# imuncle/TSCM_Calib

Hardware: AMD Instinct MI355X
Metric: LM iterations/sec at 4 cams x 10k views (joint intrinsics+extrinsics, fp64) (higher is better)
Workload: dtype f64

## Files before the change

### tscm_calib_amd/csrc/tscm_kernels.h

```cpp
#pragma once

#include "tscm_math.h"
#include "tscm_fastmath.h"
#include "tscm_nd_plan.h"
#include "tscm_layout.h"
#include "tscm_exec_plan.h"
#include "tscm_columns.h"

namespace tscm {

static_assert(kColFree == kFA && kColGrad == kFR, "tscm_columns.h plans the columns of tscm_math.h's camera tile");
constexpr int kWcolTc = 3;
constexpr int kFac = 56;
constexpr int kFacM = 0;
constexpr int kFacC = 15;
constexpr int kFacL = 21;
constexpr int kFacI = 36;
constexpr int kFacZ = 42;
constexpr int kFacD = 48;
constexpr int kTcols = 15;
constexpr int kTcWb = 0, kTcWc = 4, kTcF = 8, kTcOne = 9, kTcXi = 10, kTcLam = 12, kTcAl = 13, kTcR = 14;
__host__ __device__ constexpr int tc_tc(int j) { return 3 + 4 * j; }
constexpr int kVConst = 27;
constexpr int kCConst = 48;
// ... 58 lines not shown
    default: __builtin_amdgcn_s_setprio(3); break;
    }
}

__device__ __forceinline__ const double *rec_w(const double *rec, int slot) { return rec + (size_t)kRecW * slot; }
__device__ __forceinline__ const double *rec_e(const double *rec, int V, int slot) { return rec + (size_t)kRecW * V + (size_t)kRecE * slot; }
__device__ __forceinline__ const double *rec_g(const double *rec, int V, int slot) { return rec + (size_t)(kRecW + kRecE) * V + (size_t)kRecG * slot; }

struct Options {
    int max_num_iterations;
    double function_tolerance, gradient_tolerance, parameter_tolerance;
    double initial_radius, max_radius, min_radius;
    double min_relative_decrease, min_lm_diagonal, max_lm_diagonal;
    int max_invalid;
    int jacobi_scaling;
};

struct IterLog {
    int iteration, step_is_valid, step_is_successful, pad;
    double cost, cost_change, gradient_max_norm, gradient_norm, step_norm, relative_decrease, radius;
};

enum TermReason { kNone = 0, kMaxIter, kGradTol, kMinRadius, kParamTol, kFuncTol, kInvalidSteps };

struct CtrlHead {
    int done, term_type, term_reason, iteration;
    int cur, lin_fail, num_successful, num_unsuccessful;
    int num_invalid, n_log, lm_iterations, fin_count;
    int fault, pad0;
    double radius, decrease_factor;
    double x_cost, x_norm, gmax, gnorm;
    double model_cam, stepsq_cam;
    double se_min, se_cur, se_ref, se_cand, se_acc_ref, se_acc_cand;
    double initial_cost;
    Options opt;
    long long t_begin, t_end;
};

struct Ctrl : CtrlHead {
    IterLog log[kMaxLog];
};

struct DevProblem {
    int C, B, n_points, V, N, n_pad;
    int n_chunks, n_pchunks, n_bids;
    int rp, half;
    int lds_wave;
    const double *board_xy;
    const int *view_cam, *view_board, *view_obs, *view_count;
    const double *obs_u, *obs_v;
    const int *chunk_vb, *chunk_ve, *chunk_cam, *cam_chunk_ptr;
    const int4 *chunk_desc;
    const int *bv_ptr;
    const int *view_slot, *slot_cam;
    const int *slot_view, *slot_board;
    const int *slow_boards;
    int n_slow;
    const int *pair_i, *pair_j;
    const int *pc_begin, *pc_end, *pc_tile;
    const int *bid_part_ptr;
    const int *pair_board;
    const int *bc_tile;
    const int4 *bc_desc;
    int n_bchunks, n_tiles;
    const unsigned char *col_ctl;
    const unsigned char *board_const;
    const unsigned char *col_active;
    const int *act_map;
    int n_act;
    int cam_pre[9];
    unsigned short cam_free[8];
    unsigned long long pair_mask;
    const int4 *solve_map;
    int cam_wg[9];
    int rank, world;
    const short *bid_lut;
    int bid_part_small[kSmallBids + 1];
    int g4_per;
};

struct DevState {
    double *cam_rt[2], *intr[2], *board_rt[2];
    double *board_pc, *cam_pc;
    double *vconst;
    double *cconst[2];
    double *rec[2];
    double *campart, *campart2;
    double *H[2], *H_stage;
    double *s_b, *s_c;
    double *fac;
    double *pairpart, *T;
    int *t_count;
    int *fac_fail;
    int *y_flag;
    double *yhat;
    double *Abig;
    double *bs_part, *st_part;
    int n_bs_blocks, n_st_blocks;
    Ctrl *ctrl;
    CtrlHead *ctrl_snap;
    int *stats_count, *stats_flag;
    struct CtlPub *ctl_pub;
};
struct CtlPub { int epoch, cur, done, pad; double radius; };

__global__ void k_pose_prep(DevProblem P, DevState S, int cand)
{
    if (S.ctrl->done) return;
    const int tgt = cand ? (S.ctrl->cur ^ 1) : S.ctrl->cur;
    const int i = blockIdx.x * blockDim.x + threadIdx.x;
    if (i < P.B) {
        double rt[6], out[kBoardConst];
        for (int k = 0; k < 6; ++k) rt[k] = S.board_rt[tgt][6 * i + k];
        board_constants(rt, out);
        for (int k = 0; k < kBoardConst; ++k) S.board_pc[(size_t)kBoardConst * i + k] = out[k];
    } else if (i < P.B + P.C) {
        const int m = i - P.B;
        double rt[6], out[kCamConst];
        for (int k = 0; k < 6; ++k) rt[k] = S.cam_rt[tgt][6 * m + k];
        camera_constants(rt, out);
        for (int k = 0; k < kCamConst; ++k) S.cam_pc[kCamConst * m + k] = out[k];
    }
}

__device__ __forceinline__ void load_view_const(const DevProblem &P, const DevState &S, int tgt, int cam, int board, ViewConst &vc)
{
    const double *bp = S.board_pc + (size_t)kBoardConst * board;
    for (int k = 0; k < 3; ++k) { vc.r1[k] = bp[k]; vc.r2[k] = bp[3 + k]; vc.tb[k] = S.board_rt[tgt][6 * board + 3 + k]; }
    for (int k = 0; k < 3; ++k) for (int q = 0; q < 6; ++q) vc.db[k][q] = bp[6 + 6 * k + q];
    const double *cp = S.cam_pc + kCamConst * cam;
    for (int k = 0; k < 9; ++k) vc.Rc[k] = cp[k];
    for (int k = 0; k < 27; ++k) vc.dRc[k] = cp[9 + k];
    for (int k = 0; k < 3; ++k) vc.tc[k] = S.cam_rt[tgt][6 * cam + 3 + k];
    const double *I = S.intr[tgt] + 9 * cam;
    vc.fx = I[0]; vc.fy = I[1]; vc.cx = I[2]; vc.cy = I[3]; vc.xi = I[4]; vc.lam = I[5]; vc.al = I[6];
}

__device__ __forceinline__ void view_point_constants(const double Rc[9], const double *tc, const double *bc , const double *tb, double *o)
{
    for (int r = 0; r < 3; ++r) {
        o[r] = Rc[3 * r] * bc[0] + Rc[3 * r + 1] * bc[1] + Rc[3 * r + 2] * bc[2];
        o[3 + r] = Rc[3 * r] * bc[3] + Rc[3 * r + 1] * bc[4] + Rc[3 * r + 2] * bc[5];
        o[6 + r] = (Rc[3 * r] * tb[0] + Rc[3 * r + 1] * tb[1] + Rc[3 * r + 2] * tb[2]) + tc[r];
    }
}

#if defined(__HIP_DEVICE_COMPILE__) && !defined(__gfx950__) && !defined(__gfx942__)
#error "the in-launch hand-offs (handoff_store / handoff_load) rely on gfx942 / gfx950 sc1 write-through semantics: re-derive them for this target"
#endif
constexpr long long kHandoffTimeoutTicks = 50 * 1000 * 1000;
__device__ __forceinline__ void handoff_store(double *p, double v) { __hip_atomic_store(p, v, __ATOMIC_RELAXED, __HIP_MEMORY_SCOPE_AGENT); }
__device__ __forceinline__ double handoff_load(const double *p) { return __hip_atomic_load(p, __ATOMIC_RELAXED, __HIP_MEMORY_SCOPE_AGENT); }

__device__ __forceinline__ void write_camera_record(const DevState &S, int tgt, int m, const double *cam_rt, const double *intr)
{
    double crt[3], Rc[9], a[9], wsm[3];
    for (int k = 0; k < 3; ++k) crt[k] = cam_rt[6 * m + k];
    const int small = camera_rotation_constants(crt, Rc, a, wsm);
    double *o = S.cconst[tgt] + kCStride * m;
    for (int k = 0; k < 9; ++k) o[k] = Rc[k];
    for (int k = 0; k < 3; ++k) o[9 + k] = cam_rt[6 * m + 3 + k];
    for (int k = 0; k < 9; ++k) o[12 + k] = a[k];
    for (int k = 0; k < 3; ++k) o[21 + k] = wsm[k];
    o[24] = small ? 1.0 : 0.0;
    for (int k = 25; k < 39; ++k) o[k] = 0.0;
    double I[7];
    for (int k = 0; k < 7; ++k) I[k] = intr[9 * m + k];
    for (int k = 0; k < 6; ++k) o[39 + k] = I[k];
    const double oma = 1.0 - I[6];
    o[45] = I[6] / oma;
    o[46] = 1.0 / (oma * oma);
    o[47] = 0.0;
    float *of = reinterpret_cast<float *>(o + kCConst);
    for (int k = 0; k < kCConst; ++k) of[k] = (float)o[k];
}
__device__ __forceinline__ void write_camera_record(const DevState &S, int tgt, int m) { write_camera_record(S, tgt, m, S.cam_rt[tgt], S.intr[tgt]); }

constexpr int kVStride = 48;
constexpr int kVFloatOff = 32;
constexpr int kVPrepThreads = 128;

__device__ __forceinline__ void view_prep_body(const DevProblem &P, const DevState &S, int tgt, int with_floats, const double *cam_rt, const double *intr, const double *board_rt)
{
    __shared__ double st[kVPrepThreads][kVFloatOff + 1];
    const int t = threadIdx.x;
    const int i = blockIdx.x * kVPrepThreads + t;
    if (i < P.V) {
        const int b = P.view_board[i], m = P.view_cam[i];
        double rt[6], bc[kBoardConst], Rc[9], dRc[27];
        for (int k = 0; k < 6; ++k) rt[k] = board_rt[6 * b + k];
        board_constants(rt, bc);
        double crt[3];
        for (int k = 0; k < 3; ++k) crt[k] = cam_rt[6 * m + k];
        rotation_and_derivatives(crt, Rc, dRc);
        double *o = st[t];
        view_point_constants(Rc, cam_rt + 6 * m + 3, bc, rt + 3, o);
        for (int k = 0; k < 6; ++k) {
            const double d0 = bc[6 + 3 * k], d1 = bc[6 + 3 * k + 1], d2 = bc[6 + 3 * k + 2];
            for (int r = 0; r < 3; ++r) o[9 + 3 * k + r] = Rc[3 * r] * d0 + Rc[3 * r + 1] * d1 + Rc[3 * r + 2] * d2;
        }
        for (int k = kVConst; k < kVFloatOff; ++k) o[k] = 0.0;
    } else if (i < P.V + P.C) {
        write_camera_record(S, tgt, i - P.V, cam_rt, intr);
    }
    __syncthreads();
    const int v0 = blockIdx.x * kVPrepThreads;
    const int nv = min(kVPrepThreads, P.V - v0);
    for (int e = t; e < nv * kVFloatOff; e += kVPrepThreads) {
        const int v = e / kVFloatOff, k = e % kVFloatOff;
        S.vconst[(size_t)kVStride * (v0 + v) + k] = st[v][k];
    }
    if (with_floats) {
        constexpr int kF = kVStride - kVFloatOff;
        for (int e = t; e < nv * kF; e += kVPrepThreads) {
            const int v = e / kF, k = e % kF, j = 2 * k;
            const float f0 = j < kVConst ? (float)st[v][j] : 0.f, f1 = j + 1 < kVConst ? (float)st[v][j + 1] : 0.f;
            S.vconst[(size_t)kVStride * (v0 + v) + kVFloatOff + k] = __hiloint2double(__float_as_int(f1), __float_as_int(f0));
        }
    }
}

__global__ __launch_bounds__(kVPrepThreads) void k_view_prep(DevProblem P, DevState S, int cand, int with_floats)
{
    if (S.ctrl->done) return;
    const int tgt = cand ? (S.ctrl->cur ^ 1) : S.ctrl->cur;
    view_prep_body(P, S, tgt, with_floats, S.cam_rt[tgt], S.intr[tgt], S.board_rt[tgt]);
}

__host__ __device__ __forceinline__ constexpr int f_tile(int f)
{
    return f < 3 ? kTcWc + f : f < 6 ? tc_tc(f - 3) : f < 8 ? kTcF : f < 10 ? kTcOne : f == 10 ? kTcXi : f == 11 ? kTcLam : f == 12 ? kTcAl : kTcR;
}
__device__ __forceinline__ int f_mask(int f) { return (f >= 6 && f < 10) ? (1 << ((f - 6) & 1)) : 3; }

typedef const double __attribute__((address_space(4))) *cptr4;

struct RecLane { unsigned off, stride, goff, gstride; };
__device__ __forceinline__ RecLane rec_lane(int lane, unsigned V)
{
    const int col = lane & 15, kq = lane >> 4;
    RecLane r;
    r.goff = col == kTcR ? 8u * ((unsigned)(kRecW + kRecE) * V + (unsigned)kq) : 0xffffe000u; r.gstride = col == kTcR ? 8u * kRecG : 0u;
    if (col < 3) { r.off = 8u * ((unsigned)kRecW * V + 6u * (unsigned)col + (unsigned)kq); r.stride = 8u * kRecE; }
    else if (col == 15) { r.off = 0xffffe000u; r.stride = 0u; }
    else {
        const int f = (col & 3) == 3 ? kWcolTc + (col >> 2) : col < 8 ? col - kTcWc : col == kTcF ? 6 : col == kTcOne ? 8 : col == kTcXi ? 10 : col - 1;
        r.off = 8u * (6u * (unsigned)f + (unsigned)kq); r.stride = 8u * kRecW;
    }
    return r;
}

template <typename PW, typename PR>
__host__ __device__ __forceinline__ double tb_tb(PW W, PR Rc, int l, int lp)
{
    double t = Rc[3 + lp] * W[6 * (kWcolTc + 1) + 3 + l];
    t = fma(Rc[lp], W[6 * kWcolTc + 3 + l], t);
    return fma(Rc[6 + lp], W[6 * (kWcolTc + 2) + 3 + l], t);
}

__device__ __forceinline__ void store_view_record(__amdgpu_buffer_rsrc_t r_rec, int lane, const d4 &accU, const d4 &accV, cptr4 cc, unsigned slot, RecLane rl)
{
    int le = lane;
    asm volatile("" : "+v"(le));
    const int col = le & 15;
    const bool k3 = le >= 48, split = col == kTcF || col == kTcOne;
    constexpr unsigned BAD = 0xffffe000u;
    const unsigned off = rl.off + __umul24(slot, rl.stride);
    const double t0 = accU[0] + accV[0], t1 = accU[1] + accV[1], t2 = accU[2] + accV[2];
    double tbT[3], tbU[3];
#pragma unroll
    for (int l = 0; l < 3; ++l) {
        tbT[l] = fma(cc[6 + l], t2, fma(cc[l], t0, cc[3 + l] * t1));
        tbU[l] = fma(cc[6 + l], accU[2], fma(cc[l], accU[0], cc[3 + l] * accU[1]));
    }
    const double selT = k3 ? tbT[0] : t0, selU = k3 ? tbU[0] : accU[0];
    buf_store_f64(r_rec, off, 0u, split ? selU : selT);
    buf_store_2f64(r_rec, (k3 ? off : BAD) + 8u, split ? tbU[1] : tbT[1], split ? tbU[2] : tbT[2]);
    buf_store_f64(r_rec, (split ? off : BAD) + 48u, 0u, selT - selU);
    buf_store_2f64(r_rec, (split && k3 ? off : BAD) + 56u, tbT[1] - tbU[1], tbT[2] - tbU[2]);
    const unsigned og = rl.goff + __umul24(slot, rl.gstride);
    buf_store_f64(r_rec, og, 0u, selT);
    buf_store_2f64(r_rec, (k3 ? og : BAD) + 8u, tbT[1], tbT[2]);
}


enum GCol { gcWb0 = 0, gcWb1, gcWb2, gcTc0, gcTc1, gcTc2, gcWc0, gcWc1, gcWc2, gcF, gcOne, gcXi, gcLam, gcAl, gcR };

template <typename FV, typename FC, typename FP>
__device__ __forceinline__ void corner_geometry(double x, double y, double ou, double ov, FV VC, FC CC, FP PUT)
{
    const double X = fma(x, VC(0), fma(y, VC(3), VC(6)));
    const double Y = fma(x, VC(1), fma(y, VC(4), VC(7)));
    const double Z = fma(x, VC(2), fma(y, VC(5), VC(8)));
    const double fx = CC(39), fy = CC(40), xi = CC(43), lam = CC(44), beta = CC(45);
    const double rho2 = X * X + Y * Y;
    double d1, id1, d2, id2, d3, id3;
    sqrt_and_inverse(rho2 + Z * Z, d1, id1);
    const double z1 = Z + xi * d1;
    sqrt_and_inverse(rho2 + z1 * z1, d2, id2);
    const double z2 = z1 + lam * d2;
    sqrt_and_inverse(rho2 + z2 * z2, d3, id3);
    const double k = z2 + beta * d3;
    const double ik = fast_rcp(k);
    const double mx = X * ik, my = Y * ik;
    const double c1 = 1.0 + xi * Z * id1;
    const double c2 = 1.0 + lam * z1 * id2;
    const double c3 = 1.0 + beta * z2 * id3;
    const double q = beta * id3 + c3 * (lam * id2 + c2 * xi * id1);
    const double kz = c1 * c2 * c3;
    const double fxk = fx * ik, fyk = fy * ik;
    const double n00 = -fxk * (1.0 - X * mx * q), n01 = fxk * mx * Y * q, n02 = fxk * mx * kz;
    const double n10 = fyk * my * X * q, n11 = -fyk * (1.0 - Y * my * q), n12 = fyk * my * kz;
    PUT(gcTc0, n00, n10);
    PUT(gcTc1, n01, n11);
    PUT(gcTc2, n02, n12);
#pragma unroll
    for (int kk = 0; kk < 3; ++kk) {
        const double h0 = x * VC(9 + 6 * kk) + y * VC(12 + 6 * kk);
        const double h1 = x * VC(10 + 6 * kk) + y * VC(13 + 6 * kk);
        const double h2 = x * VC(11 + 6 * kk) + y * VC(14 + 6 * kk);
        PUT(gcWb0 + kk, n00 * h0 + n01 * h1 + n02 * h2, n10 * h0 + n11 * h1 + n12 * h2);
    }
    {
        double Q0 = X - CC(9), Q1 = Y - CC(10), Q2 = Z - CC(11);
        if (CC(24) != 0.0) {
            const double w0 = CC(21), w1 = CC(22), w2 = CC(23);
            const double s0 = w1 * Q2 - w2 * Q1, s1 = w2 * Q0 - w0 * Q2, s2 = w0 * Q1 - w1 * Q0;
// ... 1080 lines not shown
        if (!factor_core(M, g, sb, radius, dmin, dmax, facl[tid], board_is_const)) *S.fac_fail = 1;
    }
    __syncthreads();
    PHASE_STAMP(ts2);
    for (int i = tid; i < nbd * kFac; i += 256) S.fac[(size_t)kFac * c0 + i] = (&facl[0][0])[i];
    d4 acc[NT];
#pragma unroll
    for (int t = 0; t < NT; ++t) acc[t] = d4{ 0.0, 0.0, 0.0, 0.0 };
    const bool grad_col = a == kFR;
#pragma unroll
    for (int g = 0; g < 4; ++g) {
        if (16 * wave + 4 * g >= nbd) break;
        const int bg = 16 * wave + 4 * g + kq;
        const bool valid = bg < nbd;
        const int bl = min(bg, nbd - 1);
        FacFwd F;
#pragma unroll
        for (int i = 0; i < 15; ++i) F.m[i] = facl[bl][kFacM + i];
#pragma unroll
        for (int i = 0; i < 6; ++i) { F.c[i] = facl[bl][kFacC + i]; F.z[i] = valid ? facl[bl][kFacZ + i] : 0.0; }
        double y[NV][6];
#pragma unroll
        for (int p = 0; p < NV; ++p) y_column(F, w[g][p], grad_col, y[p]);
#pragma unroll
        for (int r = 0; r < 6; ++r) {
            int t = 0;
#pragma unroll
            for (int p = 0; p < NV; ++p)
#pragma unroll
                for (int q = p; q < NV; ++q, ++t) acc[t] = __builtin_amdgcn_mfma_f64_16x16x4f64(y[p][r], y[q][r], acc[t], 0, 0, 0);
        }
    }
    PHASE_STAMP(ts3);
#pragma unroll
    for (int t = 0; t < NT; ++t)
#pragma unroll
        for (int r = 0; r < 4; ++r) tiles[wave][t][(kq + 4 * r) * 16 + a] = acc[t][r];
    __syncthreads();
#pragma unroll
    for (int t = 0; t < NT; ++t)
        S.pairpart[(size_t)256 * P.bc_tile[6 * chunk + t] + tid] = (tiles[0][t][tid] + tiles[1][t][tid]) + (tiles[2][t][tid] + tiles[3][t][tid]);
#ifdef TSCM_WAVE_TIMELINE
    if (threadIdx.x == 0 && ktl_scope.on && (int)blockIdx.x < kKtlGroups) {
        long long *o = g_phs + (size_t)kPhStamps * blockIdx.x;
        o[0] = tsk; o[1] = ts0; o[2] = ts1; o[3] = ts2; o[4] = ts3; o[5] = wall_clock64(); o[6] = nbd; o[7] = (bid >= first_round ? 1 : 0) | ((RIDE && t_waited ? t_waited - tsk : 0) << 1) | ((RIDE && t_reduced ? t_reduced - tsk : 0) << 32);
    }
#endif
#ifdef TSCM_PHASE_PROFILE
    if (threadIdx.x == 0 && (cblk == 0 || cblk == 200))
        printf("schur_gram wg %d: boards %d  head %lld  E sums %lld  factor %lld  gram %lld  tiles %lld [10 ns]\n", (int)blockIdx.x, nbd, ts0 - tsk, ts1 - ts0, ts2 - ts1, ts3 - ts2, wall_clock64() - ts3);
#endif
}

__global__ __launch_bounds__(256) void k_pair_gram(DevProblem P, DevState S)
{
    if (S.ctrl->done) return;
    __shared__ double red[4][256];
    const int pc = blockIdx.x;
    const int cur = S.ctrl->cur;
    const int wave = threadIdx.x >> 6, lane = threadIdx.x & 63;
    const int a = lane & 15, kq = lane >> 4;
    d4 acc = { 0.0, 0.0, 0.0, 0.0 };
    for (int p = P.pc_begin[pc] + wave; p < P.pc_end[pc]; p += 4) {
        const double *Wi = rec_w(S.rec[cur], P.pair_i[p]), *Wj = rec_w(S.rec[cur], P.pair_j[p]);
        FacFwd F;
        load_fac_fwd(S.fac, __builtin_amdgcn_readfirstlane(P.pair_board[p]), F);
        double wi[6], wj[6];
#pragma unroll
        for (int k = 0; k < 6; ++k) { wi[k] = a < 14 ? Wi[6 * a + k] : 0.0; wj[k] = a < 14 ? Wj[6 * a + k] : 0.0; }
        double i0, i1, j0, j1;
        y_column_operands(F, wi, a == kFR, kq, i0, i1);
        y_column_operands(F, wj, a == kFR, kq, j0, j1);
        acc = __builtin_amdgcn_mfma_f64_16x16x4f64(i0, j0, acc, 0, 0, 0);
        acc = __builtin_amdgcn_mfma_f64_16x16x4f64(i1, j1, acc, 0, 0, 0);
    }
#pragma unroll
    for (int r = 0; r < 4; ++r) red[wave][(kq + 4 * r) * 16 + a] = acc[r];
    __syncthreads();
    const int t = threadIdx.x;
    S.pairpart[(size_t)256 * P.pc_tile[pc] + t] = (red[0][t] + red[1][t]) + (red[2][t] + red[3][t]);
}

constexpr int kTEntries = 64;
template <int ENTRIES>
__device__ __forceinline__ void t_reduce_block(const DevState &S, int bid, int part, int cb, int ce, double (*red)[ENTRIES])
{
    const int e = threadIdx.x % ENTRIES, slice = threadIdx.x / ENTRIES;
    const int entry = part * ENTRIES + e;
    const int per = (ce - cb + kTSlices - 1) / kTSlices;
    const int b0 = cb + slice * per, b1 = min(ce, b0 + per);
    double a0 = 0.0, a1 = 0.0, a2 = 0.0, a3 = 0.0, a4 = 0.0, a5 = 0.0, a6 = 0.0, a7 = 0.0;
    const double *src = S.pairpart + entry;
    for (int c = b0; c < b1; c += 8) {
        const double v0 = src[(size_t)256 * c];
        const double v1 = c + 1 < b1 ? src[(size_t)256 * (c + 1)] : 0.0;
        const double v2 = c + 2 < b1 ? src[(size_t)256 * (c + 2)] : 0.0;
        const double v3 = c + 3 < b1 ? src[(size_t)256 * (c + 3)] : 0.0;
        const double v4 = c + 4 < b1 ? src[(size_t)256 * (c + 4)] : 0.0;
        const double v5 = c + 5 < b1 ? src[(size_t)256 * (c + 5)] : 0.0;
        const double v6 = c + 6 < b1 ? src[(size_t)256 * (c + 6)] : 0.0;
        const double v7 = c + 7 < b1 ? src[(size_t)256 * (c + 7)] : 0.0;
        a0 += v0; a1 += v1; a2 += v2; a3 += v3; a4 += v4; a5 += v5; a6 += v6; a7 += v7;
    }
    red[slice][e] = ((a0 + a1) + (a2 + a3)) + ((a4 + a5) + (a6 + a7));
    __syncthreads();
    if (slice == 0) {
        double v[kTSlices];
#pragma unroll
        for (int q = 0; q < kTSlices; ++q) v[q] = red[q][e];
#pragma unroll
        for (int w = kTSlices / 2; w >= 1; w >>= 1)
#pragma unroll
            for (int q = 0; q < w; ++q) v[q] += v[q + w];
        handoff_store(&S.T[(size_t)256 * bid + entry], v[0]);
    }
}
__global__ __launch_bounds__(kTEntries * kTSlices) void k_T_reduce(DevProblem P, DevState S)
{
    if (S.ctrl->done) return;
    __shared__ double red[kTSlices][kTEntries];
    constexpr int kParts = 256 / kTEntries;
    const int bid = blockIdx.x / kParts;
    t_reduce_block<kTEntries>(S, bid, blockIdx.x % kParts, P.bid_part_ptr[bid], P.bid_part_ptr[bid + 1], red);
}

__device__ __forceinline__ double load_T_lut(const DevProblem &P, const double *T, int i, int j)
{
    int lo = i >> 4, hi = j >> 4, a = i & 15, b = j & 15;
    if (lo > hi) { const int t = lo; lo = hi; hi = t; const int u = a; a = b; b = u; }
    const int tile = P.bid_lut[lo * P.C + hi];
    return tile >= 0 ? T[(size_t)256 * tile + a * 16 + b] : 0.0;
}

struct TailOperands { double x, hg, hrow[kFA]; };
__device__ __forceinline__ void tail_prefetch(const DevProblem &P, const DevState &S, int cur, const double *H, TailOperands &o)
{
    const int i = threadIdx.x;
    o.x = 0.0; o.hg = 0.0;
#pragma unroll
    for (int b = 0; b < kFA; ++b) o.hrow[b] = 0.0;
    if (i < P.n_pad) {
        const int m = i >> 4, ai = i & 15;
        if (ai < 6) o.x = S.cam_rt[cur][6 * m + ai];
        else if (ai < 15) o.x = S.intr[cur][9 * m + (ai - 6)];
        if (ai < kFA) {
#pragma unroll
            for (int b = 0; b < kFA; ++b) o.hrow[b] = H[256 * m + ai * 16 + b];
            o.hg = H[256 * m + ai * 16 + kFR];
        }
    }
}
__device__ __forceinline__ void reduced_solution_tail(const DevProblem &P, const DevState &S, int cur, int fail, const TailOperands &o,
                                                      const double *yv, const double *s_sc, double *s_yh, const unsigned char *s_act, double *sred,
                                                      int publish_epoch = 0)
{
    const int n = P.n_pad, i = threadIdx.x;
    const int m = i >> 4, ai = i & 15;
    double model = 0.0, stepsq = 0.0, yh = 0.0;
    if (i < n) {
        const bool act = s_act[i] && !fail;
        yh = act ? s_sc[i] * yv[i] : 0.0;
        handoff_store(&S.yhat[i], yh);
        s_yh[i] = yh;
        if (ai < kFA) {
            const double x = o.x;
            const double xn = x + (-yh);
            if (ai < 6) handoff_store(&S.cam_rt[cur ^ 1][6 * m + ai], xn); else handoff_store(&S.intr[cur ^ 1][9 * m + (ai - 6)], xn);
            const double d = x - xn; stepsq = d * d;
        } else if (ai < 15) {
            handoff_store(&S.intr[cur ^ 1][9 * m + (ai - 6)], o.x);
        }
    }
    if (publish_epoch > 0) asm volatile("s_waitcnt vmcnt(0)" ::: "memory");
    __syncthreads();
    if (publish_epoch > 0 && i == 0) __hip_atomic_store(S.y_flag, 2 * publish_epoch + (fail ? 1 : 0), __ATOMIC_RELAXED, __HIP_MEMORY_SCOPE_AGENT);
    if (publish_epoch > 0 && i >= 64 && i < 64 + P.C) write_camera_record(S, cur ^ 1, i - 64);
    if (i < n && ai < kFA && yh != 0.0) {
        double hy = 0.0;
#pragma unroll
        for (int b = 0; b < kFA; ++b) hy += o.hrow[b] * s_yh[m * 16 + b];
        model = yh * (o.hg - 0.5 * hy);
    }
    { double red[2] = { model, stepsq }, mdummy = 0.0; block_reduce256<2>(red, mdummy, sred); model = red[0]; stepsq = red[1]; }
    if (i == 0) { S.ctrl->model_cam = model; S.ctrl->stepsq_cam = stepsq; S.ctrl->lin_fail = fail; *S.fac_fail = 0; }
}

template <int NTH, bool WAIT>
__device__ __forceinline__ void backsub_body(const DevProblem &P, const DevState &S, int with_floats, const int blk, const int nblk, const int epoch, const int t_need);

#include "tscm_solve_nd.h"
#include "tscm_solve_dense4.h"

constexpr int kBigNT = 1024;
constexpr int kBigBatch = 4;
__host__ __device__ inline size_t solve_big_lds_bytes(int N, int n_pad)
{
    return sizeof(double) * ((size_t)2 * 16 * (N + 16) + 16 * 17 + 2 * (size_t)N + 16 + 3 * (size_t)n_pad) + sizeof(int) * (size_t)N + (size_t)n_pad;
}
__device__ __forceinline__ size_t big_block(int I, int J) { return ((size_t)(I * (I + 1) / 2 + J)) << 8; }
__device__ __forceinline__ size_t big_idx(int r, int c)
{
    return big_block(r >> 4, c >> 4) + (size_t)((((c & 15) + 16 * (r & 3)) << 2) + ((r & 15) >> 2));
}
__device__ __forceinline__ double readlane_f64(double v, int lane)
{
    return __hiloint2double(__builtin_amdgcn_readlane(__double2hiint(v), lane), __builtin_amdgcn_readlane(__double2loint(v), lane));
}
__device__ __forceinline__ void lds_barrier() { asm volatile("s_waitcnt lgkmcnt(0)\n\ts_barrier" ::: "memory"); }

__global__ __launch_bounds__(kBigNT) void k_solve_reduced_big(DevProblem P, DevState S)
{
    extern __shared__ __attribute__((aligned(32))) double lds[];
    const int n = P.n_pad, na = P.n_act;
    const int N = (na + 15) & ~15, NP = N >> 4;
    const int XP = N + 16;
    double *pbuf = lds;
    double *Ld = pbuf + 2 * 16 * XP;
    double *wv = Ld + 16 * 17;
    double *idg = wv + N;
    double *yk = idg + N;
    double *yv = yk + 16;
    double *s_sc = yv + n;
    double *s_yh = s_sc + n;
    int *s_map = reinterpret_cast<int *>(s_yh + n);
    unsigned char *s_act = reinterpret_cast<unsigned char *>(s_map + N);
    __shared__ int s_fail;
    __shared__ double sred[256];
    const int tid = threadIdx.x, wave = tid >> 6, lane = tid & 63;
    if (S.ctrl->done) return;
    const int cur = S.ctrl->cur;
    const double radius = S.ctrl->radius;
    const double dmin = S.ctrl->opt.min_lm_diagonal, dmax = S.ctrl->opt.max_lm_diagonal;
    const double *H = S.H[cur];
    double *A = S.Abig;
    for (int i = tid; i < n; i += kBigNT) { s_sc[i] = S.s_c[i]; s_act[i] = P.col_active[i]; yv[i] = 0.0; }
    for (int i = tid; i < N; i += kBigNT) s_map[i] = i < na ? P.act_map[i] : -1;
    if (tid == 0) s_fail = S.ctrl->lin_fail | *S.fac_fail;
    __syncthreads();
#ifdef TSCM_BIG_PROFILE
    long long tp0 = wall_clock64(), tp_diag = 0, tp_solve = 0, tp_upd = 0;
#endif
    for (int kb = 0; wave + 16 * kb <= N; kb += 16) {
        const int rmax = min(N, wave + 16 * (kb + 15));
        for (int c = lane; c <= rmax && c < N; c += 64) {
            const int j = s_map[c];
            const int mj = j >> 4, bj = j & 15;
            const double scj = j >= 0 ? s_sc[j] : 0.0;
            double v[16];
#pragma unroll
            for (int u = 0; u < 16; ++u) {
                const int r = wave + 16 * (kb + u);
                v[u] = (r == c) ? 1.0 : 0.0;
                if (r > N || c > r) continue;
                if (r == N) {
                    v[u] = j >= 0 ? scj * (H[256 * mj + bj * 16 + kFR] - load_T_lut(P, S.T, j, mj * 16 + kFR)) : 0.0;
                } else {
                    const int i = s_map[r];
                    if (i >= 0 && j >= 0) {
                        const int mi = i >> 4, ai = i & 15;
                        const double h = (mi == mj) ? H[256 * mi + ai * 16 + bj] : 0.0;
                        double t = s_sc[i] * scj * (h - load_T_lut(P, S.T, i, j));
                        if (i == j) t += fmin(fmax(scj * scj * h, dmin), dmax) / radius;
                        v[u] = t;
                    }
                }
            }
#pragma unroll
            for (int u = 0; u < 16; ++u) {
                const int r = wave + 16 * (kb + u);
                if (r > N || c > r) continue;
                if (c < 16) pbuf[c * XP + r] = v[u];
                else A[big_idx(r, c)] = v[u];
            }
        }
    }
    __syncthreads();
#ifdef TSCM_BIG_PROFILE
    long long tp1 = wall_clock64();
#endif
    for (int tk = 0; tk < NP; ++tk) {
        const int k0 = tk * 16, m0 = k0 + 16;
        double *pc = pbuf + (tk & 1) * (16 * XP);
        double *pn = pbuf + ((tk & 1) ^ 1) * (16 * XP);
#ifdef TSCM_BIG_PROFILE
        const long long q0 = wall_clock64();
#endif
        if (wave == 0) {
            const int r = lane & 15;
            double a[16];
#pragma unroll
            for (int c = 0; c < 16; ++c) a[c] = pc[c * XP + r];
#pragma unroll
            for (int c = 0; c < 16; ++c) {
                double d = readlane_f64(a[c], c);
                if (!(d > 0.0)) { d = 1.0; if (lane == 0) s_fail = 1; }
                const double isd = fast_rsqrt(d);
                const double l = a[c] * isd;
                a[c] = l;
                if (lane == c) idg[k0 + c] = isd;
#pragma unroll
                for (int q = c + 1; q < 16; ++q) a[q] -= l * readlane_f64(l, q);
            }
            if (lane < 16) {
#pragma unroll
                for (int c = 0; c < 16; ++c) if (c <= r) { Ld[r * 17 + c] = a[c]; A[big_idx(k0 + r, k0 + c)] = a[c]; }
            }
        }
        lds_barrier();
#ifdef TSCM_BIG_PROFILE
        const long long q1 = wall_clock64();
#endif
        for (int r = m0 + tid; r <= N; r += kBigNT) {
            double x[16];
#pragma unroll
            for (int c = 0; c < 16; ++c) x[c] = pc[c * XP + (r - k0)];
#pragma unroll
            for (int c = 0; c < 16; ++c) {
                double v = x[c];
#pragma unroll
                for (int q = 0; q < c; ++q) v -= x[q] * Ld[c * 17 + q];
                x[c] = v * idg[k0 + c];
            }
#pragma unroll
            for (int c = 0; c < 16; ++c) { A[big_idx(r, k0 + c)] = x[c]; pc[c * XP + (r - k0)] = x[c]; }
        }
        lds_barrier();
#ifdef TSCM_BIG_PROFILE
        const long long q2 = wall_clock64();
#endif
        {
            const int col = lane & 15, kq = lane >> 4;
            const int Tb = tk + 1;
            for (int I = Tb + (((wave >> 2) - Tb) & 3); I <= NP; I += 4) {
                double xa[4];
#pragma unroll
                for (int t = 0; t < 4; ++t) xa[t] = -pc[(4 * t + kq) * XP + (16 * I - k0) + col];
                for (int J0 = Tb + (((wave & 3) - Tb) & 3); J0 <= I && J0 < NP; J0 += 4 * kBigBatch) {
                    d4 acc[kBigBatch];
#pragma unroll
                    for (int u = 0; u < kBigBatch; ++u) {
                        const int J = J0 + 4 * u;
                        const int Jc = (J <= I && J < NP) ? J : J0;
                        acc[u] = *reinterpret_cast<const d4 *>(A + big_block(I, Jc) + 4 * lane);
                    }
#pragma unroll
                    for (int u = 0; u < kBigBatch; ++u) {
                        const int J = J0 + 4 * u;
                        if (!(J <= I && J < NP)) continue;
                        double xb[4];
#pragma unroll
                        for (int t = 0; t < 4; ++t) xb[t] = pc[(4 * t + kq) * XP + (16 * J - k0) + col];
#pragma unroll
                        for (int t = 0; t < 4; ++t) acc[u] = __builtin_amdgcn_mfma_f64_16x16x4f64(xa[t], xb[t], acc[u], 0, 0, 0);
                    }
#pragma unroll
                    for (int u = 0; u < kBigBatch; ++u) {
                        const int J = J0 + 4 * u;
                        if (!(J <= I && J < NP)) continue;
                        if (J == Tb) {
// ... 562 lines not shown
```

### tscm_calib_amd/csrc/tscm_solve_dense4.h

```cpp
#pragma once

__device__ __forceinline__ double load_T_small(const DevProblem &P, const double *T, int i, int j)
{
    int lo = i >> 4, hi = j >> 4, a = i & 15, b = j & 15;
    if (lo > hi) { const int t = lo; lo = hi; hi = t; const int u = a; a = b; b = u; }
    const int bit = lo * 8 + hi;
    const unsigned long long m = P.pair_mask;
    const int tile = __popcll(m & ((1ull << bit) - 1ull));
    return ((m >> bit) & 1ull) ? T[256 * tile + a * 16 + b] : 0.0;
}

__host__ __device__ __forceinline__ int kth_set_bit16(unsigned w, int k)
{
    int pos = 0, c;
    c = __builtin_popcount(w & 0xffu); if (k >= c) { k -= c; w >>= 8; pos += 8; }
    c = __builtin_popcount(w & 0xfu);  if (k >= c) { k -= c; w >>= 4; pos += 4; }
    c = __builtin_popcount(w & 0x3u);  if (k >= c) { k -= c; w >>= 2; pos += 2; }
    c = (int)(w & 1u);                 if (k >= c) pos += 1;
    return pos;
}
__device__ __forceinline__ int compact_to_padded(const DevProblem &P, int ci)
{
    int base = 0, q0 = 0;
    unsigned w = P.cam_free[0];
#pragma unroll
    for (int q = 1; q < kMaxCamLds; ++q) { const bool ge = ci >= P.cam_pre[q]; base = ge ? P.cam_pre[q] : base; q0 = ge ? q : q0; w = ge ? P.cam_free[q] : w; }
    return ci < P.n_act ? 16 * q0 + kth_set_bit16(w, ci - base) : -1;
}
template <int TS, int G = 16, int NPD = 64, bool FUSED = false>
__global__ __launch_bounds__((G * G + 63) / 64 * 64, FUSED ? 3 : 1) void k_solve_reduced(DevProblem P, DevState S, int epoch, int withhold, int n_prod, int n_bs, int with_floats)
{
    constexpr int NT = (G * G + 63) / 64 * 64;
    if constexpr (FUSED) {
        static_assert(NT == kFusedEntries * kTSlices, "the T reduction runs in the solver's workgroup shape");
        if ((int)blockIdx.x > n_prod) {
#ifdef TSCM_WAVE_TIMELINE
            KtlScope ktl_bs(5, S.ctrl);
            ktl_bs.blk = (int)blockIdx.x - 1 - n_prod;
#endif
            backsub_body<256, true>(P, S, with_floats, (int)blockIdx.x - 1 - n_prod, n_bs, epoch, epoch * n_prod);
            return;
        }
    }
    KTL(4);
    if constexpr (FUSED) {
        if (blockIdx.x > 0) {
            constexpr int kParts = 256 / kFusedEntries;
            const int bid = ((int)blockIdx.x - 1) / kParts, part = ((int)blockIdx.x - 1) % kParts;
            const int cb = P.bid_part_small[bid], ce = P.bid_part_small[bid + 1];
            if (S.ctrl->done) return;
            __shared__ double red[kTSlices][kFusedEntries];
            t_reduce_block<kFusedEntries>(S, bid, part, cb, ce, red);
            asm volatile("s_waitcnt vmcnt(0)" ::: "memory");
            __syncthreads();
            if (threadIdx.x == 0 && !(withhold && blockIdx.x == 1))
                __hip_atomic_fetch_add(S.t_count, 1, __ATOMIC_RELAXED, __HIP_MEMORY_SCOPE_AGENT);
            return;
        }
    }
    PHASE_STAMP(ts0);
    const int ctrl_done = S.ctrl->done;
    constexpr int N = G * TS;
    constexpr int LD = N + 2;
    extern __shared__ __attribute__((aligned(16))) double lds[];
    double *Lm = lds;
    constexpr int XT = TS * TS + 2;
    double *Xb = Lm + N * LD;
    double *wp = Xb + 2 * G * XT;
    double *idg = wp + N;
    double *yv = idg + N;
    double *s_sc = yv + NPD;
    double *s_yh = s_sc + NPD;
    __shared__ int s_fail;
    __shared__ unsigned char s_act[NPD];
    __shared__ double sred[256];
    const int n = P.n_pad;
    const int tid = threadIdx.x;
    const int NP = (P.n_act + TS - 1) / TS;
    int off[kSolveMapSlots];
#pragma unroll
    for (int q = 0; q < kSolveMapSlots / 4; ++q) {
        const int4 v = P.solve_map[q * NT + tid];
        off[4 * q] = v.x; off[4 * q + 1] = v.y; off[4 * q + 2] = v.z; off[4 * q + 3] = v.w;
    }
    const int ri = off[kMapTile], cj = off[kMapTile + 1];
    const bool mine = off[kMapTile + 2] == 1, rhsrow = off[kMapTile + 2] == 2;
    const int cur = S.ctrl->cur;
    const double radius = S.ctrl->radius;
    const double dmin = S.ctrl->opt.min_lm_diagonal, dmax = S.ctrl->opt.max_lm_diagonal;
    const int ctrl_fail = S.ctrl->lin_fail | *S.fac_fail;
    for (int i = tid; i < NPD; i += NT) { s_sc[i] = i < n ? S.s_c[i] : 1.0; s_act[i] = i < n ? P.col_active[i] : 0; yv[i] = 0.0; }
    if (ctrl_done) return;
    const double *H = S.H[cur];
    double sci[TS], scj[TS], hh[TS][TS], tt[TS][TS];
#pragma unroll
    for (int r = 0; r < TS; ++r) {
        const int oi = off[kMapSci + r], oj = off[kMapScj + r];
        sci[r] = oi == kMapOne ? 1.0 : oi >= 0 ? S.s_c[oi] : 0.0;
        scj[r] = oj >= 0 ? S.s_c[oj] : 0.0;
    }
#pragma unroll
    for (int r = 0; r < TS; ++r)
#pragma unroll
        for (int c = 0; c < TS; ++c) { const int oh = off[kMapH + r * TS + c]; hh[r][c] = oh >= 0 ? H[oh] : 0.0; }
    if constexpr (FUSED) {
        __shared__ int s_late;
        if (tid == 0) {
            const int need = epoch * n_prod;
            const long long t_start = wall_clock64();
            int late = 0;
            while (__hip_atomic_load(S.t_count, __ATOMIC_RELAXED, __HIP_MEMORY_SCOPE_AGENT) < need) {
                __builtin_amdgcn_s_sleep(2);
                if (wall_clock64() - t_start > kHandoffTimeoutTicks) { late = 1; break; }
            }
            __builtin_amdgcn_fence(__ATOMIC_ACQUIRE, "agent");
            if (late) {
                S.ctrl->fault = 1; S.ctrl->term_type = 2; S.ctrl->done = 1;
                __builtin_amdgcn_fence(__ATOMIC_RELEASE, "agent");
                if (n_bs > 0) __hip_atomic_store(S.y_flag, 2 * epoch + 1, __ATOMIC_RELAXED, __HIP_MEMORY_SCOPE_AGENT);
            }
            s_late = late;
        }
        __syncthreads();
        if (s_late) return;
    }
#pragma unroll
    for (int r = 0; r < TS; ++r)
#pragma unroll
        for (int c = 0; c < TS; ++c) { const int ot = off[kMapT + r * TS + c]; tt[r][c] = ot >= 0 ? (FUSED ? handoff_load(&S.T[ot]) : S.T[ot]) : 0.0; }
    PHASE_STAMP(ts0b);
    if (tid == 0) s_fail = ctrl_fail;
    double a[TS][TS];
    const double inv_radius = 1.0 / radius;
#pragma unroll
    for (int r = 0; r < TS; ++r) {
#pragma unroll
        for (int c = 0; c < TS; ++c) {
            const bool dg = mine && ri == cj && r == c;
            double v = sci[r] * scj[c] * (hh[r][c] - tt[r][c]);
            if (dg) v = (off[kMapSci + r] >= 0 && off[kMapSci + r] != kMapOne) ? v + fmin(fmax(sci[r] * sci[r] * hh[r][c], dmin), dmax) * inv_radius : 1.0;
            a[r][c] = v;
        }
    }
    PHASE_STAMP(ts1);
#ifdef TSCM_PHASE_PROFILE
    const long long cy1 = clock64();
#endif
    auto publish_tile = [&](double *dst, const double (&t)[TS][TS]) {
#pragma unroll
        for (int r = 0; r < TS; ++r)
#pragma unroll
            for (int c = 0; c < TS; ++c) dst[r * TS + c] = t[r][c];
    };
    auto factor_diag = [&](double (&t)[TS][TS], int tk) {
        double il[TS];
#pragma unroll
        for (int c = 0; c < TS; ++c) {
            double d = t[c][c];
#pragma unroll
            for (int q = 0; q < c; ++q) d -= t[c][q] * t[c][q];
            if (!(d > 0.0)) { s_fail = 1; d = 1.0; }
            const double isd = fast_rsqrt(d);
            t[c][c] = d * isd; il[c] = isd;
#pragma unroll
            for (int r = c + 1; r < TS; ++r) {
                double v = t[r][c];
#pragma unroll
                for (int q = 0; q < c; ++q) v -= t[r][q] * t[c][q];
                t[r][c] = v * isd;
            }
        }
#pragma unroll
        for (int r = 0; r < TS; ++r) {
            idg[tk * TS + r] = il[r];
#pragma unroll
            for (int c = 0; c < TS; ++c) Lm[(tk * TS + r) * LD + tk * TS + c] = c <= r ? t[r][c] : 0.0;
        }
    };
    struct PanelFactor { double l[TS][TS], il[TS]; };
    auto load_factor = [&](PanelFactor &f, int tk) {
#pragma unroll
        for (int r = 0; r < TS; ++r) {
            f.il[r] = idg[tk * TS + r];
#pragma unroll
            for (int c = 0; c < TS; ++c) f.l[r][c] = Lm[(tk * TS + r) * LD + tk * TS + c];
        }
    };
    auto load_tile = [&](const double *src, double (&t)[TS][TS]) {
#pragma unroll
        for (int r = 0; r < TS; ++r)
#pragma unroll
            for (int c = 0; c < TS; ++c) t[r][c] = src[r * TS + c];
    };
    auto panel_solve = [&](const double (&At)[TS][TS], const PanelFactor &f, double (&x)[TS][TS]) {
#pragma unroll
        for (int r = 0; r < TS; ++r)
#pragma unroll
            for (int c = 0; c < TS; ++c) {
                double v = At[r][c];
#pragma unroll
                for (int q = 0; q < c; ++q) v -= x[r][q] * f.l[c][q];
                x[r][c] = v * f.il[c];
            }
    };
    __shared__ __attribute__((aligned(16))) double s_dt[2][TS * TS];
    const bool dthread = tid == NT - 1;
    if (cj == 0 && ri > 0 && (mine || rhsrow)) publish_tile(Xb + ri * XT, a);
    if (ri == 1 && cj == 1 && mine) publish_tile(s_dt[0], a);
    if (tid == 0 && NP > 0) factor_diag(a, 0);
    __syncthreads();
    for (int tk = 0; tk < NP; ++tk) {
        const double *Ar = Xb + (tk & 1) * (G * XT);
        double *ArN = Xb + ((tk + 1) & 1) * (G * XT);
#ifdef TSCM_PHASE_PROFILE
        __shared__ long long s_ph[8];
        if (tk == 3 && (dthread || tid == 11 * G + 5)) s_ph[dthread ? 0 : 4] = wall_clock64();
#endif
        if (dthread && tk + 1 < NP) {
            PanelFactor f;
            double araw[TS][TS], dt[TS][TS], x[TS][TS], t[TS][TS];
            load_factor(f, tk);
            load_tile(Ar + (tk + 1) * XT, araw);
            load_tile(s_dt[tk & 1], dt);
            __builtin_amdgcn_sched_barrier(0);
            panel_solve(araw, f, x);
#pragma unroll
            for (int r = 0; r < TS; ++r)
#pragma unroll
                for (int c = 0; c <= r; ++c) {
                    double v = dt[r][c];
#pragma unroll
                    for (int q = 0; q < TS; ++q) v -= x[r][q] * x[c][q];
                    t[r][c] = v;
                }
#ifdef TSCM_PHASE_PROFILE
            if (tk == 3) { asm volatile("" : "+v"(t[3][3])); s_ph[1] = wall_clock64(); }
#endif
            factor_diag(t, tk + 1);
#ifdef TSCM_PHASE_PROFILE
            if (tk == 3) s_ph[2] = wall_clock64();
#endif
        }
        if ((mine || rhsrow) && ri > tk && cj >= tk && !(ri == cj && ri == tk + 1)) {
            PanelFactor f;
            double ai[TS][TS], aj[TS][TS], xi[TS][TS];
            load_factor(f, tk);
            load_tile(Ar + ri * XT, ai);
            load_tile(Ar + cj * XT, aj);
            __builtin_amdgcn_sched_barrier(0);
            panel_solve(ai, f, xi);
            if (cj == tk) {
#pragma unroll
                for (int r = 0; r < TS; ++r)
#pragma unroll
                    for (int c = 0; c < TS; ++c) a[r][c] = xi[r][c];
                if (rhsrow) {
#pragma unroll
                    for (int c = 0; c < TS; ++c) wp[tk * TS + c] = xi[0][c];
                }
            } else {
                double xj[TS][TS];
                panel_solve(aj, f, xj);
#pragma unroll
                for (int r = 0; r < TS; ++r)
#pragma unroll
                    for (int c = 0; c < TS; ++c) {
                        double v = a[r][c];
#pragma unroll
                        for (int q = 0; q < TS; ++q) v -= xi[r][q] * xj[c][q];
                        a[r][c] = v;
                    }
            }
        }
        {
            const bool col = cj == tk + 1 && ri > tk + 1 && (mine || rhsrow), dg = ri == tk + 2 && cj == tk + 2 && mine;
            if (col || dg) publish_tile(col ? ArN + ri * XT : s_dt[(tk + 1) & 1], a);
        }
#ifdef TSCM_PHASE_PROFILE
        if (tk == 3 && tid == 11 * G + 5) { asm volatile("" : "+v"(a[3][3])); s_ph[5] = wall_clock64(); }
        if (tk + 1 < NP) __syncthreads();
        if (tk == 3 && tid == 0) { s_ph[6] = wall_clock64(); printf("  panel 3: D x,t %lld  factor %lld | update %lld | to barrier exit %lld\n", s_ph[1] - s_ph[0], s_ph[2] - s_ph[1], s_ph[5] - s_ph[4], s_ph[6] - s_ph[0]); }
#else
        if (tk + 1 < NP) __syncthreads();
#endif
    }
    if (cj < ri && mine) {
#pragma unroll
        for (int r = 0; r < TS; ++r)
#pragma unroll
            for (int c = 0; c < TS; ++c) Lm[(ri * TS + r) * LD + cj * TS + c] = a[r][c];
    }
    __syncthreads();
    PHASE_STAMP(ts2);
#ifdef TSCM_PHASE_PROFILE
    const long long cy2 = clock64();
#endif
    TailOperands tail_ops;
    tail_prefetch(P, S, cur, H, tail_ops);
    if (tid < 64) {
        constexpr int R = (N + 63) / 64;
        double w[R];
#pragma unroll
        for (int q = 0; q < R; ++q) w[q] = tid + 64 * q < NP * TS ? wp[tid + 64 * q] : 0.0;
        for (int tk = NP - 1; tk >= 0; --tk) {
            const int k0 = tk * TS;
            double y[TS];
#pragma unroll
            for (int c = 0; c < TS; ++c) {
                const int k = k0 + c;
                double v = 0.0;
#pragma unroll
                for (int q = 0; q < R; ++q) if ((k >> 6) == q) v = w[q];
                y[c] = __shfl(v, k & 63);
            }
#pragma unroll
            for (int c = TS - 1; c >= 0; --c) {
                double v = y[c];
#pragma unroll
                for (int q = c + 1; q < TS; ++q) v -= Lm[(k0 + q) * LD + k0 + c] * y[q];
                y[c] = v * idg[k0 + c];
            }
#pragma unroll
            for (int q = 0; q < R; ++q) {
                const int i = tid + 64 * q;
                if (i < k0) {
                    double v = w[q];
#pragma unroll
                    for (int c = 0; c < TS; ++c) v -= Lm[(k0 + c) * LD + i] * y[c];
                    w[q] = v;
                } else if (i < k0 + TS) {
#pragma unroll
                    for (int c = 0; c < TS; ++c) if (i == k0 + c) w[q] = y[c];
                }
            }
        }
#pragma unroll
        for (int q = 0; q < R; ++q) { const int pi = tid + 64 * q < N ? compact_to_padded(P, tid + 64 * q) : -1; if (pi >= 0) yv[pi] = w[q]; }
    }
    __syncthreads();
    PHASE_STAMP(ts3);
    reduced_solution_tail(P, S, cur, s_fail, tail_ops, yv, s_sc, s_yh, s_act, sred, FUSED && n_bs > 0 ? epoch : 0);
#ifdef TSCM_PHASE_PROFILE
    if (tid == 0) printf("solve_reduced: ctrl %lld operands %lld  factor %lld (%lld shader clocks)  backsub %lld  tail %lld [10 ns]\n", ts0b - ts0, ts1 - ts0b, ts2 - ts1, cy2 - cy1, ts3 - ts2, wall_clock64() - ts3);
#endif
}
```

Before: 8823.

## Software-pipeline reduced back-substitution and build camera records from LDS parameters

The back-substitution loop in the dense reduced solver now double-buffers its LDS operands, loading the next tile's triangular entries, inverse diagonals and column values while the current tile is processed. The y broadcast uses readlane instead of a shuffle. The compact-to-padded index mapping is hoisted out of the solve, with the camera-free masks pinned to scalar registers. The solution tail keeps the updated parameters in LDS and builds the camera records from them instead of re-reading global memory. Each piece targets latency on a serial, single-wave critical path, in exchange for more registers and more complex code.

```diff
diff --git a/tscm_calib_amd/csrc/tscm_kernels.h b/tscm_calib_amd/csrc/tscm_kernels.h
--- a/tscm_calib_amd/csrc/tscm_kernels.h
+++ b/tscm_calib_amd/csrc/tscm_kernels.h
@@ -234,20 +234,20 @@
 __device__ __forceinline__ void handoff_store(double *p, double v) { __hip_atomic_store(p, v, __ATOMIC_RELAXED, __HIP_MEMORY_SCOPE_AGENT); }
 __device__ __forceinline__ double handoff_load(const double *p) { return __hip_atomic_load(p, __ATOMIC_RELAXED, __HIP_MEMORY_SCOPE_AGENT); }
 
-__device__ __forceinline__ void write_camera_record(const DevState &S, int tgt, int m, const double *cam_rt, const double *intr)
+__device__ __forceinline__ void write_camera_record_at(const DevState &S, int tgt, int m, const double *rt, const double *I9)
 {
     double crt[3], Rc[9], a[9], wsm[3];
-    for (int k = 0; k < 3; ++k) crt[k] = cam_rt[6 * m + k];
+    for (int k = 0; k < 3; ++k) crt[k] = rt[k];
     const int small = camera_rotation_constants(crt, Rc, a, wsm);
     double *o = S.cconst[tgt] + kCStride * m;
     for (int k = 0; k < 9; ++k) o[k] = Rc[k];
-    for (int k = 0; k < 3; ++k) o[9 + k] = cam_rt[6 * m + 3 + k];
+    for (int k = 0; k < 3; ++k) o[9 + k] = rt[3 + k];
     for (int k = 0; k < 9; ++k) o[12 + k] = a[k];
     for (int k = 0; k < 3; ++k) o[21 + k] = wsm[k];
     o[24] = small ? 1.0 : 0.0;
     for (int k = 25; k < 39; ++k) o[k] = 0.0;
     double I[7];
-    for (int k = 0; k < 7; ++k) I[k] = intr[9 * m + k];
+    for (int k = 0; k < 7; ++k) I[k] = I9[k];
     for (int k = 0; k < 6; ++k) o[39 + k] = I[k];
     const double oma = 1.0 - I[6];
     o[45] = I[6] / oma;
@@ -255,6 +255,10 @@
     o[47] = 0.0;
     float *of = reinterpret_cast<float *>(o + kCConst);
     for (int k = 0; k < kCConst; ++k) of[k] = (float)o[k];
+}
+__device__ __forceinline__ void write_camera_record(const DevState &S, int tgt, int m, const double *cam_rt, const double *intr)
+{
+    write_camera_record_at(S, tgt, m, cam_rt + 6 * m, intr + 9 * m);
 }
 __device__ __forceinline__ void write_camera_record(const DevState &S, int tgt, int m) { write_camera_record(S, tgt, m, S.cam_rt[tgt], S.intr[tgt]); }
 
@@ -1641,7 +1645,7 @@
 }
 __device__ __forceinline__ void reduced_solution_tail(const DevProblem &P, const DevState &S, int cur, int fail, const TailOperands &o,
                                                       const double *yv, const double *s_sc, double *s_yh, const unsigned char *s_act, double *sred,
-                                                      int publish_epoch = 0)
+                                                      int publish_epoch = 0, double *s_par = nullptr)
 {
     const int n = P.n_pad, i = threadIdx.x;
     const int m = i >> 4, ai = i & 15;
@@ -1655,15 +1659,21 @@
             const double x = o.x;
             const double xn = x + (-yh);
             if (ai < 6) handoff_store(&S.cam_rt[cur ^ 1][6 * m + ai], xn); else handoff_store(&S.intr[cur ^ 1][9 * m + (ai - 6)], xn);
+            if (s_par) s_par[i] = xn;
             const double d = x - xn; stepsq = d * d;
         } else if (ai < 15) {
             handoff_store(&S.intr[cur ^ 1][9 * m + (ai - 6)], o.x);
+            if (s_par) s_par[i] = o.x;
         }
     }
     if (publish_epoch > 0) asm volatile("s_waitcnt vmcnt(0)" ::: "memory");
     __syncthreads();
     if (publish_epoch > 0 && i == 0) __hip_atomic_store(S.y_flag, 2 * publish_epoch + (fail ? 1 : 0), __ATOMIC_RELAXED, __HIP_MEMORY_SCOPE_AGENT);
-    if (publish_epoch > 0 && i >= 64 && i < 64 + P.C) write_camera_record(S, cur ^ 1, i - 64);
+    if (publish_epoch > 0 && i >= 64 && i < 64 + P.C) {
+        const int c = i - 64;
+        if (s_par) write_camera_record_at(S, cur ^ 1, c, s_par + 16 * c, s_par + 16 * c + 6);
+        else write_camera_record(S, cur ^ 1, c);
+    }
     if (i < n && ai < kFA && yh != 0.0) {
         double hy = 0.0;
 #pragma unroll
@@ -1676,6 +1686,11 @@
 
 template <int NTH, bool WAIT>
 __device__ __forceinline__ void backsub_body(const DevProblem &P, const DevState &S, int with_floats, const int blk, const int nblk, const int epoch, const int t_need);
+
+__device__ __forceinline__ double readlane_f64(double v, int lane)
+{
+    return __hiloint2double(__builtin_amdgcn_readlane(__double2hiint(v), lane), __builtin_amdgcn_readlane(__double2loint(v), lane));
+}
 
 #include "tscm_solve_nd.h"
 #include "tscm_solve_dense4.h"
@@ -1690,10 +1705,6 @@
 __device__ __forceinline__ size_t big_idx(int r, int c)
 {
     return big_block(r >> 4, c >> 4) + (size_t)((((c & 15) + 16 * (r & 3)) << 2) + ((r & 15) >> 2));
-}
-__device__ __forceinline__ double readlane_f64(double v, int lane)
-{
-    return __hiloint2double(__builtin_amdgcn_readlane(__double2hiint(v), lane), __builtin_amdgcn_readlane(__double2loint(v), lane));
 }
 __device__ __forceinline__ void lds_barrier() { asm volatile("s_waitcnt lgkmcnt(0)\n\ts_barrier" ::: "memory"); }
 
diff --git a/tscm_calib_amd/csrc/tscm_solve_dense4.h b/tscm_calib_amd/csrc/tscm_solve_dense4.h
--- a/tscm_calib_amd/csrc/tscm_solve_dense4.h
+++ b/tscm_calib_amd/csrc/tscm_solve_dense4.h
@@ -21,10 +21,13 @@
 }
 __device__ __forceinline__ int compact_to_padded(const DevProblem &P, int ci)
 {
+    unsigned cf[kMaxCamLds];
+#pragma unroll
+    for (int q = 0; q < kMaxCamLds; ++q) { cf[q] = P.cam_free[q]; asm volatile("" : "+s"(cf[q])); }
     int base = 0, q0 = 0;
-    unsigned w = P.cam_free[0];
-#pragma unroll
-    for (int q = 1; q < kMaxCamLds; ++q) { const bool ge = ci >= P.cam_pre[q]; base = ge ? P.cam_pre[q] : base; q0 = ge ? q : q0; w = ge ? P.cam_free[q] : w; }
+    unsigned w = cf[0];
+#pragma unroll
+    for (int q = 1; q < kMaxCamLds; ++q) { const bool ge = ci >= P.cam_pre[q]; base = ge ? P.cam_pre[q] : base; q0 = ge ? q : q0; w = ge ? cf[q] : w; }
     return ci < P.n_act ? 16 * q0 + kth_set_bit16(w, ci - base) : -1;
 }
 template <int TS, int G = 16, int NPD = 64, bool FUSED = false>
@@ -128,6 +131,10 @@
     for (int r = 0; r < TS; ++r)
 #pragma unroll
         for (int c = 0; c < TS; ++c) { const int ot = off[kMapT + r * TS + c]; tt[r][c] = ot >= 0 ? (FUSED ? handoff_load(&S.T[ot]) : S.T[ot]) : 0.0; }
+    constexpr int R = (N + 63) / 64;
+    int pcol[R];
+#pragma unroll
+    for (int q = 0; q < R; ++q) pcol[q] = tid < 64 && tid + 64 * q < N ? compact_to_padded(P, tid + 64 * q) : -1;
     PHASE_STAMP(ts0b);
     if (tid == 0) s_fail = ctrl_fail;
     double a[TS][TS];
@@ -298,11 +305,24 @@
     TailOperands tail_ops;
     tail_prefetch(P, S, cur, H, tail_ops);
     if (tid < 64) {
-        constexpr int R = (N + 63) / 64;
         double w[R];
 #pragma unroll
         for (int q = 0; q < R; ++q) w[q] = tid + 64 * q < NP * TS ? wp[tid + 64 * q] : 0.0;
-        for (int tk = NP - 1; tk >= 0; --tk) {
+        struct BsOps { double u[TS][TS], id[TS], col[R][TS]; };
+        auto bs_load = [&](BsOps &o, int tk) {
+            const int k0 = tk * TS;
+#pragma unroll
+            for (int c = 0; c < TS; ++c) {
+                o.id[c] = idg[k0 + c];
+#pragma unroll
+                for (int q = c + 1; q < TS; ++q) o.u[c][q] = Lm[(k0 + q) * LD + k0 + c];
+            }
+#pragma unroll
+            for (int q = 0; q < R; ++q)
+#pragma unroll
+                for (int c = 0; c < TS; ++c) o.col[q][c] = Lm[(k0 + c) * LD + min(tid + 64 * q, N - 1)];
+        };
+        auto bs_step = [&](int tk, const BsOps &o) {
             const int k0 = tk * TS;
             double y[TS];
 #pragma unroll
@@ -311,14 +331,14 @@
                 double v = 0.0;
 #pragma unroll
                 for (int q = 0; q < R; ++q) if ((k >> 6) == q) v = w[q];
-                y[c] = __shfl(v, k & 63);
+                y[c] = readlane_f64(v, k & 63);
             }
 #pragma unroll
             for (int c = TS - 1; c >= 0; --c) {
                 double v = y[c];
 #pragma unroll
-                for (int q = c + 1; q < TS; ++q) v -= Lm[(k0 + q) * LD + k0 + c] * y[q];
-                y[c] = v * idg[k0 + c];
+                for (int q = c + 1; q < TS; ++q) v -= o.u[c][q] * y[q];
+                y[c] = v * o.id[c];
             }
 #pragma unroll
             for (int q = 0; q < R; ++q) {
@@ -326,20 +346,29 @@
                 if (i < k0) {
                     double v = w[q];
 #pragma unroll
-                    for (int c = 0; c < TS; ++c) v -= Lm[(k0 + c) * LD + i] * y[c];
+                    for (int c = 0; c < TS; ++c) v -= o.col[q][c] * y[c];
                     w[q] = v;
                 } else if (i < k0 + TS) {
 #pragma unroll
                     for (int c = 0; c < TS; ++c) if (i == k0 + c) w[q] = y[c];
                 }
             }
-        }
-#pragma unroll
-        for (int q = 0; q < R; ++q) { const int pi = tid + 64 * q < N ? compact_to_padded(P, tid + 64 * q) : -1; if (pi >= 0) yv[pi] = w[q]; }
+        };
+        BsOps oa, ob;
+        bs_load(oa, max(NP - 1, 0));
+        for (int tk = NP - 1; tk >= 0; tk -= 2) {
+            bs_load(ob, max(tk - 1, 0));
+            bs_step(tk, oa);
+            if (tk == 0) break;
+            bs_load(oa, max(tk - 2, 0));
+            bs_step(tk - 1, ob);
+        }
+#pragma unroll
+        for (int q = 0; q < R; ++q) if (pcol[q] >= 0) yv[pcol[q]] = w[q];
     }
     __syncthreads();
     PHASE_STAMP(ts3);
-    reduced_solution_tail(P, S, cur, s_fail, tail_ops, yv, s_sc, s_yh, s_act, sred, FUSED && n_bs > 0 ? epoch : 0);
+    reduced_solution_tail(P, S, cur, s_fail, tail_ops, yv, s_sc, s_yh, s_act, sred, FUSED && n_bs > 0 ? epoch : 0, yv);
 #ifdef TSCM_PHASE_PROFILE
     if (tid == 0) printf("solve_reduced: ctrl %lld operands %lld  factor %lld (%lld shader clocks)  backsub %lld  tail %lld [10 ns]\n", ts0b - ts0, ts1 - ts0b, ts2 - ts1, cy2 - cy1, ts3 - ts2, wall_clock64() - ts3);
 #endif
```

Result: no change. 8864 (median of 6 runs) (+0.5%).
